# jaxsonpd/air_rs

Hardware: AMD Instinct MI355X
Metric: IQ Msamples/s (decoded Mode-S msgs/s alongside), 2 MSPS i8 stream (higher is better)
Workload: dtype i8; 1 GPU; 2 MSPS i8 IQ, 1 GiB synthetic buffer per GPU, fused magnitude+preamble/DF17 gate+PPM+CRC-24; samples_per_gpu=536870912, bytes_per_gpu=1073741824, channels=1

## Files before the change

### air_rs_amd/csrc/adsb_api.cpp

```cpp
#include <hip/hip_runtime.h>

#include <algorithm>
#include <chrono>
#include <cstdio>
#include <cstdlib>
#include <cmath>
#include <cstring>
#include <new>
#include <vector>

#include "adsb_kernels.h"
#include "adsb_synth.h"

using adsbk::kTile;
using adsbk::kWindow;

namespace {
constexpr int kTimingRing = 512;
}

struct adsb_ctx {
    adsb_cfg cfg{};
    hipStream_t stream = nullptr;
    bool own_stream = false;
// ... 227 lines not shown
        }
        const size_t n_slots = (size_t)c->n_tiles_max * adsbk::kQuota + c->cap_slots;
        bool ok = true;
        for (auto &r : c->rs) {
            ok = ok && hipMalloc((void **)&r.seg, sizeof(adsbk::Seg) * (size_t)c->n_tiles_max) == hipSuccess &&
                 hipMalloc((void **)&r.slots, sizeof(adsb_frame) * n_slots) == hipSuccess &&
                 hipMalloc((void **)&r.out, sizeof(adsb_frame) * (size_t)cfg->max_out) == hipSuccess &&
                 hipMalloc((void **)&r.hdr, sizeof(adsbk::Header)) == hipSuccess &&
                 hipMalloc((void **)&r.chan_prefix, sizeof(uint64_t) * ((size_t)cfg->max_channels + 1)) == hipSuccess &&
                 hipMemsetAsync(r.chan_prefix, 0, sizeof(uint64_t) * ((size_t)cfg->max_channels + 1), c->stream) == hipSuccess &&
                 hipEventCreateWithFlags(&r.k_done, hipEventDisableTiming | hipEventReleaseToDevice) == hipSuccess &&
                 hipEventCreateWithFlags(&r.g_done, hipEventDisableTiming | hipEventReleaseToDevice) == hipSuccess &&
                 hipMemsetAsync(r.hdr, 0, sizeof(adsbk::Header), c->stream) == hipSuccess;
        }
        c->lb_groups_at = (uint32_t)(((size_t)c->n_tiles_max / adsbk::kFinishTilesPerWg + 2 + 63) / 64 * 64);
        const size_t lb_words = (size_t)c->lb_groups_at + c->lb_groups_at / 64 + 64;
        ok = ok && hipMalloc((void **)&c->out_start, sizeof(uint32_t) * ((size_t)c->n_tiles_max + 1)) == hipSuccess &&
             hipMalloc((void **)&c->scratch, 64) == hipSuccess &&
             hipMalloc((void **)&c->lb, sizeof(uint64_t) * lb_words) == hipSuccess &&
             hipMemsetAsync(c->lb, 0, sizeof(uint64_t) * lb_words, c->stream) == hipSuccess &&
             hipMemsetAsync(c->scratch, 0, 64, c->stream) == hipSuccess;
        if (!ok) { fail(ADSB_E_NOMEM); break; }
        if (hipHostMalloc((void **)&c->hdr_host, sizeof(adsbk::Header), hipHostMallocDefault) != hipSuccess) { fail(ADSB_E_NOMEM); break; }
        uint32_t probe[4] = {0, 0, 0, 0};
        e = adsbk::probe_cvt(c->stream, c->scratch, probe);
        if (e != hipSuccess) { fail((int)e); break; }
        const uint32_t want = 0u | (2u << 8) | (180u << 16);
        if (probe[0] == want) c->mag_mode = 0;
        else if (probe[1] == want) c->mag_mode = 1;
        else c->mag_mode = 2;
        if (const char *force = getenv("ADSB_FORCE_MAG_MODE")) c->mag_mode = atoi(force) % 3;
        if (c->scan == adsbk::kScanCode) {
            std::vector<uint16_t> tab(32769);
            const int prc = code_table_check(c, tab.data());
            if (prc != ADSB_OK) { fail(prc); break; }
        }
        c->stamps_bytes = adsbk::tile_stamps_built() ? (size_t)c->n_tiles_max * 64 + 512 : 512;
        if (hipMalloc((void **)&c->stamps, c->stamps_bytes) != hipSuccess || hipMemsetAsync(c->stamps, 0, c->stamps_bytes, c->stream) != hipSuccess) { fail(ADSB_E_NOMEM); break; }
    } while (0);
    if (rc != ADSB_OK) { adsb_destroy(c); return rc; }
    *out_ctx = c;
    return ADSB_OK;
}

extern "C" void *adsb_stream(adsb_ctx *c) { return c ? (void *)c->stream : nullptr; }
extern "C" int adsb_sample_type(const adsb_ctx *c) { return c ? c->cfg.sample_type : ADSB_E_ARG; }
extern "C" int adsb_debug_fused_pass_only(adsb_ctx *c, int on)
{
    if (!c) return ADSB_E_ARG;
    c->fused_pass_only = on != 0;
    return ADSB_OK;
}
extern "C" int adsb_debug_mag_mode(adsb_ctx *c) { return c ? c->mag_mode : ADSB_E_ARG; }
extern "C" int adsb_debug_scan(adsb_ctx *c) { return c ? (c->cfg.sample_type == ADSB_SAMPLE_I8 ? c->scan : adsbk::kScanRoot) : ADSB_E_ARG; }
// ... 1921 lines not shown
```

### air_rs_amd/csrc/adsb_kernels.h

```cpp
#pragma once
#include <hip/hip_runtime.h>
#include <stddef.h>
#include <stdint.h>

#include "../../include/adsb_hip.h"

namespace adsbk {

#ifndef ADSB_KRUN
#define ADSB_KRUN 32
#endif
#ifndef ADSB_THREADS
#define ADSB_THREADS 256
#endif
constexpr int kThreads = ADSB_THREADS;
constexpr int kRun = ADSB_KRUN;
constexpr int kTile = 2 * kThreads * kRun;
constexpr int kHalo = 256;
constexpr int kMag = kTile + kHalo;
#ifndef ADSB_KRUN_I16
#define ADSB_KRUN_I16 16
#endif
constexpr int kRunI16 = ADSB_KRUN_I16;
template <int ST> struct TileCfg {
    static constexpr int kRunT = ST == ADSB_SAMPLE_I8 ? kRun : kRunI16;
    static constexpr int kTileT = 2 * kThreads * kRunT;
    static constexpr int kMagT = kTileT + kHalo;
};
constexpr int tile_offsets(int sample_type)
{
    return sample_type == ADSB_SAMPLE_I8 ? kTile : 2 * kThreads * kRunI16;
}
constexpr int kTileMax = kTile > 2 * kThreads * kRunI16 ? kTile : 2 * kThreads * kRunI16;
constexpr int kScanNsq = 0, kScanRoot = 1, kScanReg = 2, kScanCode = 3, kScanSieve = 4;
constexpr int kRegTile = 4 * 2 * 63 * 32;
#ifndef ADSB_SV_SWEEPS
#define ADSB_SV_SWEEPS 8
#endif
constexpr int kSieveTile = ADSB_SV_SWEEPS * kThreads * 8;
constexpr int tile_offsets_of(int sample_type, int scan)
{
    return (sample_type == ADSB_SAMPLE_I8 && scan == kScanReg) ? kRegTile
           : (sample_type == ADSB_SAMPLE_I8 && scan == kScanSieve) ? kSieveTile : tile_offsets(sample_type);
}
constexpr int kListCap = 128;
constexpr int kSparseCap = 64;
constexpr int kWindow = 240;
constexpr uint32_t kNoBase = 0xFFFFFFFFu;
constexpr uint32_t kQuota = 32;
struct Seg {
    uint32_t base;
    uint32_t cand;
    uint32_t valid;
    uint32_t decoded;
};

struct Header {
    uint64_t n_out;
    uint64_t total_found;
    uint32_t flags;
    uint32_t retry;
    unsigned long long alloc;
};

struct DemodArgs {
    const void *iq;
// ... 19 lines not shown
    Seg *seg;
    adsb_frame *slots;
    adsb_frame *out;
    const uint32_t *out_start;
    uint64_t *lb;
    uint32_t lb_groups_at;
    uint64_t *chan_prefix;
    uint32_t epoch;
    uint32_t tiles_per_channel;
    uint32_t n_channels;
    uint32_t max_out;
    uint32_t tile_first, tile_count;
    Header *hdr;
    uint64_t *hdr_pub;
    uint32_t stall_blk;
};

struct SmallArgs {
    uint32_t *done;
    uint64_t *seq_host;
    uint64_t seq;
};

hipError_t probe_cvt(hipStream_t s, uint32_t *dev_scratch4, uint32_t host_out[4]);
hipError_t launch_code_probe(hipStream_t s, uint16_t *dev_out32769);

hipError_t launch_demod(hipStream_t s, int sample_type, int mag_mode, int scan, const DemodArgs &a,
                        hipEvent_t e0 = nullptr, hipEvent_t e1 = nullptr);
hipError_t launch_finish(hipStream_t s, const FinishArgs &a, hipEvent_t e0 = nullptr, hipEvent_t e1 = nullptr);
hipError_t launch_empty_result(hipStream_t s, Header *hdr, uint64_t *hdr_pub, uint64_t *chan_prefix, uint32_t n_channels,
                               hipEvent_t e0 = nullptr, hipEvent_t e1 = nullptr);
constexpr int kFinishTilesPerWg = 32;
hipError_t launch_small(hipStream_t s, int sample_type, int mag_mode, int scan, const DemodArgs &p, const FinishArgs &f,
                        const SmallArgs &sm);

bool ab_kernels_built();
bool tile_stamps_built();

hipError_t launch_decode_fields(hipStream_t s, const adsb_frame *frames, const Header *hdr, uint32_t cap,
                                adsb_packet_fields *out);

struct TrackRecord {
    adsb_aircraft_record a;
    double t_even, t_odd;
    uint32_t even_lat, even_lon, odd_lat, odd_lon;
    uint32_t have;
    uint32_t pad;
// ... 110 lines not shown
```

### air_rs_amd/csrc/adsb_kernels.hip

```cpp
#include <hip/hip_ext.h>
#include <utility>
#include <cstdlib>

#include "adsb_kernels.h"
#include "adsb_synth.h"

namespace adsbk {

typedef unsigned int u32x4 __attribute__((ext_vector_type(4)));
typedef unsigned short u16x2 __attribute__((ext_vector_type(2)));

__device__ __forceinline__ uint32_t pkmin(uint32_t a, uint32_t b)
{
    u16x2 r = __builtin_elementwise_min(__builtin_bit_cast(u16x2, a), __builtin_bit_cast(u16x2, b));
    return __builtin_bit_cast(uint32_t, r);
}
__device__ __forceinline__ uint32_t pkmax(uint32_t a, uint32_t b)
{
    u16x2 r = __builtin_elementwise_max(__builtin_bit_cast(u16x2, a), __builtin_bit_cast(u16x2, b));
    return __builtin_bit_cast(uint32_t, r);
}
typedef _Float16 f16x2 __attribute__((ext_vector_type(2)));
template <bool F16> __device__ __forceinline__ uint32_t pkmax3(uint32_t a, uint32_t b, uint32_t c)
{
// ... 13 lines not shown
            __builtin_bit_cast(f16x2, c));
        return __builtin_bit_cast(uint32_t, r);
    }
    return pkmin(pkmin(a, b), c);
}

__device__ __forceinline__ void dot4x8_sacc(u32x4 v, int c, int n[8])
{
    const uint32_t a0 = v.x & 0xFFFFu, a1 = v.x & 0xFFFF0000u, a2 = v.y & 0xFFFFu, a3 = v.y & 0xFFFF0000u,
                   a4 = v.z & 0xFFFFu, a5 = v.z & 0xFFFF0000u, a6 = v.w & 0xFFFFu, a7 = v.w & 0xFFFF0000u;
    asm("v_dot4_i32_i8 %0, %8, %12, %20\n\t"
        "v_dot4_i32_i8 %1, %8, %13, %20\n\t"
        "v_dot4_i32_i8 %2, %9, %14, %20\n\t"
        "v_dot4_i32_i8 %3, %9, %15, %20\n\t"
        "v_dot4_i32_i8 %4, %10, %16, %20\n\t"
        "v_dot4_i32_i8 %5, %10, %17, %20\n\t"
        "v_dot4_i32_i8 %6, %11, %18, %20\n\t"
        "v_dot4_i32_i8 %7, %11, %19, %20\n\t"
        "s_nop 2"
        : "=&v"(n[0]), "=&v"(n[1]), "=&v"(n[2]), "=&v"(n[3]), "=&v"(n[4]), "=&v"(n[5]), "=&v"(n[6]), "=&v"(n[7])
        : "v"(v.x), "v"(v.y), "v"(v.z), "v"(v.w), "v"(a0), "v"(a1), "v"(a2), "v"(a3), "v"(a4), "v"(a5),
          "v"(a6), "v"(a7), "s"(c));
}

struct SynTable {
    uint32_t v[112];
};
constexpr SynTable make_syn()
{
    SynTable t{};
    uint32_t r = 1;
    for (int e = 0; e < 112; ++e) {
        t.v[111 - e] = r;
        r <<= 1;
        if (r & 0x1000000u) r ^= 0x1FFF409u;
    }
    return t;
}
__constant__ SynTable kSyn = make_syn();

template <int MAGMODE> __device__ __forceinline__ float mag_root_i8(int n_plus_2p23)
{
    float f = __builtin_bit_cast(float, n_plus_2p23) - 8388607.5f;
    float r = __builtin_amdgcn_sqrtf(f);
    if (MAGMODE == 2) r -= 0.5f;
    return r;
}

typedef float f32x2 __attribute__((ext_vector_type(2)));
template <int MAGMODE>
__device__ __forceinline__ void mags8_i8(u32x4 v, uint32_t &lo, uint32_t &hi)
{
    int n[8];
    dot4x8_sacc(v, 0x4B000000, n);
    float f[8];
#pragma unroll
    for (int k = 0; k < 8; k += 2) {
        f32x2 t = {__builtin_bit_cast(float, n[k]), __builtin_bit_cast(float, n[k + 1])};
        t = t - (f32x2){8388607.5f, 8388607.5f};
        f[k] = t.x;
        f[k + 1] = t.y;
    }
    float r[8];
#pragma unroll
    for (int k = 0; k < 8; ++k) {
        r[k] = __builtin_amdgcn_sqrtf(f[k]);
        if (MAGMODE == 2) r[k] -= 0.5f;
    }
    lo = __builtin_amdgcn_cvt_pk_u8_f32(r[0], 0, 0u);
    lo = __builtin_amdgcn_cvt_pk_u8_f32(r[1], 1, lo);
    lo = __builtin_amdgcn_cvt_pk_u8_f32(r[2], 2, lo);
    lo = __builtin_amdgcn_cvt_pk_u8_f32(r[3], 3, lo);
    hi = __builtin_amdgcn_cvt_pk_u8_f32(r[4], 0, 0u);
    hi = __builtin_amdgcn_cvt_pk_u8_f32(r[5], 1, hi);
    hi = __builtin_amdgcn_cvt_pk_u8_f32(r[6], 2, hi);
    hi = __builtin_amdgcn_cvt_pk_u8_f32(r[7], 3, hi);
}

__device__ __forceinline__ uint32_t mag_i16_fix(uint32_t r, uint32_t n)
{
    return r - ((__umul24(r, r) > n) ? 1u : 0u);
}
__device__ __forceinline__ uint32_t mag_i16(uint32_t iq)
{
    uint32_t n, r;
    asm("v_dot2_i32_i16 %0, %2, %2, 0\n\t"
        "s_nop 2\n\t"
        "v_cvt_f32_u32 %1, %0\n\t"
        "v_sqrt_f32 %1, %1\n\t"
        "s_nop 0\n\t"
        "v_cvt_rpi_i32_f32 %1, %1"
        : "=&v"(n), "=&v"(r)
        : "v"(iq));
    return mag_i16_fix(r, n);
}
__device__ __forceinline__ void mags4_i16(u32x4 v, uint32_t &lo, uint32_t &hi)
{
    uint32_t n0, n1, n2, n3, r0, r1, r2, r3;
    asm("v_dot2_i32_i16 %0, %8, %8, 0\n\t"
// ... 19 lines not shown
        : "v"(v.x), "v"(v.y), "v"(v.z), "v"(v.w));
    lo = __builtin_amdgcn_perm(mag_i16_fix(r1, n1), mag_i16_fix(r0, n0), 0x05040100u);
    hi = __builtin_amdgcn_perm(mag_i16_fix(r3, n3), mag_i16_fix(r2, n2), 0x05040100u);
}

__global__ void probe_cvt_kernel(uint32_t *out)
{
    if (threadIdx.x != 0) return;
    float a = 0.75f, b = 2.5f, c = 180.9986f;
    asm volatile("" : "+v"(a), "+v"(b), "+v"(c));
    uint32_t r0 = __builtin_amdgcn_cvt_pk_u8_f32(a, 0, 0u);
    r0 = __builtin_amdgcn_cvt_pk_u8_f32(b, 1, r0);
    r0 = __builtin_amdgcn_cvt_pk_u8_f32(c, 2, r0);
    out[0] = r0;
    __builtin_amdgcn_s_setreg((1 | (0 << 6) | ((2 - 1) << 11)), 3);
    asm volatile("" : "+v"(a), "+v"(b), "+v"(c));
    uint32_t r1 = __builtin_amdgcn_cvt_pk_u8_f32(a, 0, 0u);
    r1 = __builtin_amdgcn_cvt_pk_u8_f32(b, 1, r1);
    r1 = __builtin_amdgcn_cvt_pk_u8_f32(c, 2, r1);
    out[1] = r1;
    __builtin_amdgcn_s_setreg((1 | (0 << 6) | ((2 - 1) << 11)), 0);
    out[2] = 0xC0DEu;
    out[3] = 0;
}

hipError_t probe_cvt(hipStream_t s, uint32_t *dev_scratch4, uint32_t host_out[4])
{
    hipLaunchKernelGGL(probe_cvt_kernel, dim3(1), dim3(64), 0, s, dev_scratch4);
    hipError_t e = hipGetLastError();
    if (e != hipSuccess) return e;
    e = hipMemcpyAsync(host_out, dev_scratch4, 16, hipMemcpyDeviceToHost, s);
    if (e != hipSuccess) return e;
    return hipStreamSynchronize(s);
}

template <int ST> struct MagT;
template <> struct MagT<ADSB_SAMPLE_I8> { typedef uint8_t type; };
template <> struct MagT<ADSB_SAMPLE_I16> { typedef uint16_t type; };

constexpr int kNsqBias = 72;
constexpr int kNsqHalf = kTile / 2;
constexpr int kNsqLog = kNsqHalf + kHalo;
#ifndef ADSB_NSQ_PAD_SHIFT
#define ADSB_NSQ_PAD_SHIFT 6
#endif
constexpr int kNsqPadShift = ADSB_NSQ_PAD_SHIFT;
__host__ __device__ constexpr uint32_t nsq_phys(uint32_t q) { return q + 4u * (q >> kNsqPadShift); }
constexpr int kNsqPhys = (int)nsq_phys(kNsqLog);
static_assert(kNsqHalf % 64 == 0 && kHalo % 64 == 0 && kRun == 32 && (kNsqPadShift == 5 || kNsqPadShift == 6),
              "nsq image: pads every 32 or 64 dwords, runs of 32");

#ifndef ADSB_MAG_PAD
#define ADSB_MAG_PAD 0
#endif
template <int ST, int SCAN> struct MagPad {
    static constexpr bool on = ADSB_MAG_PAD != 0 && ST == ADSB_SAMPLE_I8 && SCAN == kScanRoot;
};
template <bool PAD> __host__ __device__ constexpr uint32_t mag_phys(uint32_t b) { return PAD ? b + 16u * (b >> 8) : b; }

template <int ST, int SCAN = kScanRoot> struct Lds {
    typedef typename MagT<ST>::type mag_t;
    static constexpr bool kNsq = ST == ADSB_SAMPLE_I8 && SCAN == kScanNsq;
    static constexpr int kMagBytes = kNsq ? kNsqPhys * 4
                                          : (int)((mag_phys<MagPad<ST, SCAN>::on>((uint32_t)TileCfg<ST>::kMagT * (uint32_t)sizeof(mag_t)) + 15u) & ~15u);
    static constexpr int kOffCand = kMagBytes;
    static constexpr int kOffList = kOffCand + 2 * kThreads * 4 * ((TileCfg<ST>::kRunT + 31) / 32);
    static constexpr int kOffMisc = kOffList + kListCap * 2;
    static constexpr int kTotal = kOffMisc + 64;
};

template <int ST>
__device__ __forceinline__ uint32_t pair_at(const uint32_t *ra, const uint32_t *rb, int k)
{
    if (ST == ADSB_SAMPLE_I8) {
        const uint32_t sel = 0x0C000C00u | (uint32_t)(k & 3) | ((uint32_t)(4 + (k & 3)) << 16);
        return __builtin_amdgcn_perm(rb[k >> 2], ra[k >> 2], sel);
    } else {
        const uint32_t sel = (k & 1) ? 0x07060302u : 0x05040100u;
        return __builtin_amdgcn_perm(rb[k >> 1], ra[k >> 1], sel);
    }
}

template <int ST>
__device__ __forceinline__ uint32_t pair_at_cold(const uint32_t *ra, const uint32_t *rb, int k)
{
    if (ST == ADSB_SAMPLE_I8) {
        const uint32_t sel = 0x0C000C00u | (uint32_t)(4 + (k & 3)) | ((uint32_t)(k & 3) << 16);
        return __builtin_amdgcn_perm(ra[k >> 2], rb[k >> 2], sel);
    } else {
// ... 186 lines not shown
#define ADSB_ABL_PHASES 3
#endif
#ifndef ADSB_ABL_NOCMP
#define ADSB_ABL_NOCMP 0
#endif
#ifndef ADSB_AB_KERNELS
#define ADSB_AB_KERNELS 0
#endif
bool ab_kernels_built() { return ADSB_AB_KERNELS != 0; }
#ifndef ADSB_PRIO
#define ADSB_PRIO 0
#endif
#ifndef ADSB_GATE_GROUP
#define ADSB_GATE_GROUP 1
#endif

template <int RUN, int NT>
__device__ __forceinline__ void gate_collect(uint32_t *candA, uint32_t *candB, uint16_t *list, uint32_t *count,
                                             const uint32_t tid, const uint32_t n_valid)
{
    constexpr int WPR = (RUN + 31) / 32;
    const uint32_t sa = tid * RUN, sb = (tid + NT) * RUN;
    const uint32_t va = n_valid > sa ? (n_valid - sa) : 0u, vb = n_valid > sb ? (n_valid - sb) : 0u;
    uint32_t words[2 * WPR];
    uint32_t nz = 0, c = 0;
#pragma unroll
    for (int k = 0; k < WPR; ++k) {
        words[k] = candA[k];
        words[WPR + k] = candB[k];
    }
    if (n_valid < (uint32_t)(2 * NT * RUN)) {
#pragma unroll
        for (int k = 0; k < WPR; ++k) {
            const uint32_t la = va > 32u * k ? va - 32u * k : 0u, lb = vb > 32u * k ? vb - 32u * k : 0u;
            words[k] &= la >= 32u ? 0xFFFFFFFFu : ((1u << la) - 1u);
            words[WPR + k] &= lb >= 32u ? 0xFFFFFFFFu : ((1u << lb) - 1u);
            candA[k] = words[k];
            candB[k] = words[WPR + k];
        }
    }
#pragma unroll
    for (int k = 0; k < 2 * WPR; ++k) {
        nz |= words[k];
        c += __builtin_popcount(words[k]);
    }
    if (nz) {
        uint32_t pos = atomicAdd(count, c);
#pragma unroll
        for (int k = 0; k < 2 * WPR; ++k) {
            uint32_t bits = words[k];
            const uint32_t base = (k < WPR ? sa : sb) + (k % WPR) * 32;
            while (bits) {
                const uint32_t b = __builtin_ctz(bits);
                bits &= bits - 1;
                if (pos < (uint32_t)kSparseCap) list[pos] = (uint16_t)(base + b);
                ++pos;
            }
        }
    }
}

struct NoHook {
    __device__ __forceinline__ void operator()() const {}
};

template <int ST, int GROUP, int RUN, int NT, int HOOK_AT = -1, class HOOK = NoHook, bool F16OK = (ST == ADSB_SAMPLE_I8), bool PAD = false>
__device__ __forceinline__ void gate_phase(const typename MagT<ST>::type *mag, uint32_t *cand, uint16_t *list,
                                           uint32_t *count, const uint32_t tid, const uint32_t n_valid,
                                           HOOK hook = HOOK())
{
    static_assert(RUN % GROUP == 0 && (RUN == 16 || RUN == 32 || RUN == 64), "steps are taken GROUP at a time; 1 or 2 bitmap words per run");
    constexpr int WPR = (RUN + 31) / 32;
    constexpr int SPG = 16 / (int)sizeof(typename MagT<ST>::type);
    uint32_t *candA = cand + WPR * tid, *candB = cand + WPR * (tid + NT);
#pragma unroll
    for (int k = 0; k < WPR; ++k) candA[k] = candB[k] = 0u;
    constexpr int kGran = (RUN + 26 + SPG - 1) / SPG + 1;
    static_assert(!PAD || (ST == ADSB_SAMPLE_I8 && RUN == 32 && (NT * RUN) % 256 == 0), "the padded image: u8 magnitudes, runs of 32 bytes");
    const u32x4 *ga = reinterpret_cast<const u32x4 *>(mag + mag_phys<PAD>(tid * RUN));
    const u32x4 *gb = reinterpret_cast<const u32x4 *>(mag + mag_phys<PAD>((tid + NT) * RUN));
    const uint32_t hop = PAD && (tid & 7u) == 7u ? 1u : 0u;
    const u32x4 *ga2 = ga + hop, *gb2 = gb + hop;
    uint32_t ra[kGran * 4], rb[kGran * 4];
    constexpr int kAhead = 48 / SPG;
#pragma unroll
    for (int g = 0; g < kAhead; ++g) {
        u32x4 a = (PAD && g >= 2) ? ga2[g] : ga[g], b = (PAD && g >= 2) ? gb2[g] : gb[g];
        ra[4 * g] = a.x; ra[4 * g + 1] = a.y; ra[4 * g + 2] = a.z; ra[4 * g + 3] = a.w;
        rb[4 * g] = b.x; rb[4 * g + 1] = b.y; rb[4 * g + 2] = b.z; rb[4 * g + 3] = b.w;
    }

    uint32_t N[RUN + 26], H2[RUN + 8], W3[RUN + 16], F[RUN + 9];
#pragma unroll
    for (int k = 0; k < 25; ++k) N[k] = pair_at<ST>(ra, rb, k);
#pragma unroll
    for (int j = 0; j < 7; ++j) H2[j] = pkmin(N[j], N[j + 2]);
#pragma unroll
    for (int j = 3; j < 13; ++j) W3[j] = pkmax3<F16OK>(N[j], N[j + 1], N[j + 2]);
#pragma unroll
    for (int j = 1; j < 8; ++j) F[j] = pkmax3<F16OK>(N[j], W3[j + 2], N[j + 5]);
// ... 55 lines not shown
    gate_collect<RUN, NT>(candA, candB, list, count, tid, n_valid);
}

template <int BPS, int MAG = kMag>
__device__ __forceinline__ u32x4 tile_rsrc_words(const DemodArgs &p, const TilePos &t, bool live)
{
    const uint64_t base = (uint64_t)(uintptr_t)((const char *)p.iq + ((uint64_t)t.ch * p.channel_stride + t.sample0) * BPS);
    const uint64_t remain = (p.n_samples - t.sample0) * BPS;
    const uint32_t nrec = remain > (uint64_t)(MAG * BPS) ? (uint32_t)(MAG * BPS) : (uint32_t)remain;
    u32x4 w;
    w.x = __builtin_amdgcn_readfirstlane((uint32_t)base);
    w.y = __builtin_amdgcn_readfirstlane((uint32_t)(base >> 32) & 0xFFFFu);
    w.z = __builtin_amdgcn_readfirstlane(live ? nrec : 0u);
    w.w = 0x00020000u;
    return w;
}

#ifndef ADSB_LOAD_AUX
#define ADSB_LOAD_AUX 2
#endif
template <int ST> struct P1 {
    static constexpr int kSPL = ST == ADSB_SAMPLE_I8 ? 8 : 4;
    static constexpr int kIters = (TileCfg<ST>::kMagT + kThreads * kSPL - 1) / (kThreads * kSPL);
};

template <int ST>
__device__ __forceinline__ void issue_tile_loads(const DemodArgs &p, const TilePos &tp, bool live, uint32_t tid,
                                                 u32x4 (&raw)[P1<ST>::kIters])
{
    constexpr int BPS = (ST == ADSB_SAMPLE_I8) ? 2 : 4;
    __amdgpu_buffer_rsrc_t rsrc = tile_rsrc<BPS, TileCfg<ST>::kMagT>(p, tp, live);
    const uint32_t wave_s0 = __builtin_amdgcn_readfirstlane(tid & ~63u) * P1<ST>::kSPL;
#pragma unroll
    for (int it = 0; it < P1<ST>::kIters; ++it)
        if ((uint32_t)it * (kThreads * P1<ST>::kSPL) + wave_s0 < (uint32_t)TileCfg<ST>::kMagT)
            raw[it] = __builtin_amdgcn_raw_buffer_load_b128(rsrc, tid * 16, (uint32_t)it * (kThreads * 16), ADSB_LOAD_AUX);
}

template <int ST, int MAGMODE, bool PAD = false>
__device__ __forceinline__ bool magnitudes_to_lds(const u32x4 (&raw)[P1<ST>::kIters], typename MagT<ST>::type *mag, uint32_t tid)
{
    uint32_t mx = 0;
    const uint32_t wave_s0 = __builtin_amdgcn_readfirstlane(tid & ~63u) * P1<ST>::kSPL;
#pragma unroll
    for (int it = 0; it < P1<ST>::kIters; ++it) {
        if ((uint32_t)it * (kThreads * P1<ST>::kSPL) + wave_s0 < (uint32_t)TileCfg<ST>::kMagT) {
            const uint32_t s = (uint32_t)it * (kThreads * P1<ST>::kSPL) + tid * P1<ST>::kSPL;
            uint32_t lo, hi;
            if (ST == ADSB_SAMPLE_I8) mags8_i8<MAGMODE>(raw[it], lo, hi);
            else {
                mags4_i16(raw[it], lo, hi);
                mx = pkmax(mx, pkmax(lo, hi));
            }
            const uint32_t sp = PAD ? s + 16u * (tid >> 5) + (uint32_t)it * (16u * (kThreads * P1<ST>::kSPL / 256)) : s;
            if (s < (uint32_t)TileCfg<ST>::kMagT) *reinterpret_cast<uint2 *>(mag + sp) = make_uint2(lo, hi);
        }
    }
    return ST == ADSB_SAMPLE_I16 && __builtin_amdgcn_ballot_w64(((mx & 0xFFFFu) >= 0x7C00u) || ((mx >> 16) >= 0x7C00u)) != 0;
}

constexpr int kNsqIters = (kNsqLog + kThreads * 8 - 1) / (kThreads * 8);
constexpr int kNsqFull = kNsqLog / (kThreads * 8);
constexpr int kNsqTail = kNsqLog % (kThreads * 8);
static_assert(kNsqIters - kNsqFull <= 1 && kNsqTail % 8 == 0, "at most one partial sweep of whole lanes");

__device__ __forceinline__ void nsq_issue_loads(const DemodArgs &p, const TilePos &tp, uint32_t tid,
                                                u32x4 (&ra)[kNsqIters], u32x4 (&rb)[kNsqIters])
{
    __amdgpu_buffer_rsrc_t rsrc = tile_rsrc<2, kMag>(p, tp, true);
#pragma unroll
    for (int it = 0; it < kNsqFull; ++it) {
        ra[it] = __builtin_amdgcn_raw_buffer_load_b128(rsrc, tid * 16, (uint32_t)it * (kThreads * 16), ADSB_LOAD_AUX);
        rb[it] = __builtin_amdgcn_raw_buffer_load_b128(rsrc, tid * 16, (uint32_t)it * (kThreads * 16) + 2 * kNsqHalf, ADSB_LOAD_AUX);
    }
    if (kNsqTail && __builtin_amdgcn_readfirstlane(tid & ~63u) * 8 < (uint32_t)kNsqTail) {
        ra[kNsqFull] = __builtin_amdgcn_raw_buffer_load_b128(rsrc, tid * 16, (uint32_t)kNsqFull * (kThreads * 16), ADSB_LOAD_AUX);
        rb[kNsqFull] = __builtin_amdgcn_raw_buffer_load_b128(rsrc, tid * 16, (uint32_t)kNsqFull * (kThreads * 16) + 2 * kNsqHalf, ADSB_LOAD_AUX);
    }
// ... 124 lines not shown
                uint32_t bit = 1u << o;
                asm("" : "+v"(bit));
                if (sa) atomicOr(candA, bit);
                if (sb) atomicOr(candB, bit);
            }
        }
    }
    gate_collect<RUN, NT>(candA, candB, list, count, tid, n_valid);
}

#ifndef ADSB_SCAN_WAVES
#define ADSB_SCAN_WAVES 4
#endif
#ifndef ADSB_REG_ABL
#define ADSB_REG_ABL 0
#endif
#ifndef ADSB_REG_WAVES
#define ADSB_REG_WAVES 5
#endif
template <int ST, int MAGMODE, int SCAN>
__device__ __forceinline__ void scan_tile(const DemodArgs &p, const uint32_t tile, const bool first, unsigned char *smem)
{
    typedef Lds<ST, SCAN> L;
    typedef TileCfg<ST> TC;
    typedef typename L::mag_t mag_t;
    constexpr bool NSQ = L::kNsq;
    static_assert(kThreads / 64 <= 4, "misc[4 + wave] must stay below misc[8]");

    mag_t *mag = reinterpret_cast<mag_t *>(smem);
    uint32_t *img = reinterpret_cast<uint32_t *>(smem);
    uint32_t *cand = reinterpret_cast<uint32_t *>(smem + L::kOffCand);
    uint16_t *list = reinterpret_cast<uint16_t *>(smem + L::kOffList);
    uint32_t *misc = reinterpret_cast<uint32_t *>(smem + L::kOffMisc);

    const uint32_t tid = threadIdx.x;
    const uint32_t lane = tid & 63, wave = tid >> 6;

#if ADSB_PRIO & 1
    __builtin_amdgcn_s_setprio(3);
#endif
    if (!NSQ && MAGMODE == 1) __builtin_amdgcn_s_setreg((1 | (0 << 6) | ((2 - 1) << 11)), 3);
#if ADSB_TILE_STAMPS
    unsigned long long ts_prev = 0;
    uint32_t ts_seg[9] = {0, 0, 0, 0, 0, 0, 0, 0, 0};
    ts_seg[7] = (uint32_t)__builtin_amdgcn_s_memrealtime();
    TSTAMP(-1);
    ts_seg[8] = (uint32_t)ts_prev;
// ... 29 lines not shown
        if constexpr (NSQ) wave_big = nsq_image_to_lds(raw_a, raw_b, img, tid);
        else wave_big = magnitudes_to_lds<ST, MAGMODE, MagPad<ST, SCAN>::on>(raw, mag, tid);
        if ((NSQ || ST == ADSB_SAMPLE_I16) && lane == 0) misc[4 + wave] = wave_big ? 1u : 0u;
        TSTAMP(1);
        __syncthreads();
        TSTAMP(2);
#if ADSB_ABL_PHASES < 2
        if (smem[tid * 64] == 0xFD && smem[tid * 64 + 1] == 0xFE && n_valid == 7) misc[12] = 1;
#else

        if constexpr (NSQ || ST == ADSB_SAMPLE_I16) {
            uint32_t any_big = 0;
#pragma unroll
            for (int w = 0; w < kThreads / 64; ++w) any_big |= misc[4 + w];
            const bool big = any_big != 0;
            if constexpr (NSQ) {
                if (!big) gate_phase_nsq<true>(img, cand, list, &misc[12], tid, n_valid);
                else gate_phase_nsq<false>(img, cand, list, &misc[12], tid, n_valid);
            } else {
                if (!big) gate_phase<ST, ADSB_GATE_GROUP, TC::kRunT, kThreads, -1, NoHook, true>(mag, cand, list, &misc[12], tid, n_valid);
                else gate_phase<ST, ADSB_GATE_GROUP, TC::kRunT, kThreads, -1, NoHook, false>(mag, cand, list, &misc[12], tid, n_valid);
            }
        } else {
            gate_phase<ST, ADSB_GATE_GROUP, TC::kRunT, kThreads, -1, NoHook, (ST == ADSB_SAMPLE_I8), MagPad<ST, SCAN>::on>(mag, cand, list, &misc[12], tid, n_valid);
        }
#endif
        TSTAMP(3);
        __syncthreads();
        TSTAMP(4);

#if ADSB_PRIO & 2
        __builtin_amdgcn_s_setprio(2);
#endif
        uint32_t total = misc[12];
#if ADSB_ABL_PHASES < 3
        if (total != 0x7FFFFFFFu) total = 0;
#endif
        const bool dense = total > (uint32_t)kSparseCap;
        constexpr int kBitsPerWord = TC::kRunT < 32 ? TC::kRunT : 32;
        u32x4 cw = {0, 0, 0, 0};
        uint32_t cnt = 0, my_first = 0;
        if (dense) {
            if (4 * tid < (uint32_t)(TC::kTileT / kBitsPerWord)) cw = reinterpret_cast<const u32x4 *>(cand)[tid];
            cnt = __builtin_popcount(cw.x) + __builtin_popcount(cw.y) + __builtin_popcount(cw.z) +
                  __builtin_popcount(cw.w);
            uint32_t incl = cnt;
#pragma unroll
// ... 1236 lines not shown
        *sm.done = 0;
        __builtin_amdgcn_fence(__ATOMIC_RELEASE, "");
        asm volatile("s_waitcnt vmcnt(0)" ::: "memory");
        __hip_atomic_store(sm.seq_host, sm.seq, __ATOMIC_RELAXED, __HIP_MEMORY_SCOPE_SYSTEM);
    }
}

hipError_t launch_small(hipStream_t s, int sample_type, int mag_mode, int scan, const DemodArgs &p, const FinishArgs &f,
                        const SmallArgs &sm)
{
    if (p.tile_count == 0 || p.tile_count > (uint32_t)kFinTiles) return hipErrorInvalidValue;
    dim3 grid(p.tile_count), block(kThreads);
    if (sample_type == ADSB_SAMPLE_I16) hipLaunchKernelGGL((demod_small<ADSB_SAMPLE_I16, 0, kScanRoot>), grid, block, 0, s, p, f, sm);
#if ADSB_AB_KERNELS
    else if (scan == kScanSieve) hipLaunchKernelGGL((demod_small<ADSB_SAMPLE_I8, 0, kScanSieve>), grid, block, 0, s, p, f, sm);
    else if (scan == kScanNsq) hipLaunchKernelGGL((demod_small<ADSB_SAMPLE_I8, 0, kScanNsq>), grid, block, 0, s, p, f, sm);
    else if (scan == kScanReg) hipLaunchKernelGGL((demod_small<ADSB_SAMPLE_I8, 0, kScanReg>), grid, block, 0, s, p, f, sm);
    else if (scan == kScanCode) hipLaunchKernelGGL((demod_small<ADSB_SAMPLE_I8, 0, kScanCode>), grid, block, 0, s, p, f, sm);
#else
    else if (scan != kScanRoot) return hipErrorInvalidValue;
#endif
    else if (mag_mode == 0) hipLaunchKernelGGL((demod_small<ADSB_SAMPLE_I8, 0, kScanRoot>), grid, block, 0, s, p, f, sm);
    else if (mag_mode == 1) hipLaunchKernelGGL((demod_small<ADSB_SAMPLE_I8, 1, kScanRoot>), grid, block, 0, s, p, f, sm);
    else hipLaunchKernelGGL((demod_small<ADSB_SAMPLE_I8, 2, kScanRoot>), grid, block, 0, s, p, f, sm);
    return hipGetLastError();
}

__global__ void empty_result_kernel(Header *hdr, uint64_t *hdr_pub, uint64_t *chan_prefix, uint32_t n_channels)
{
    if (threadIdx.x == 0) {
        hdr->n_out = 0;
        hdr->total_found = 0;
        hdr->flags = 0;
        hdr->retry = 0;
        hdr->alloc = 0;
        if (hdr_pub) { hdr_pub[0] = 0; hdr_pub[1] = 0; hdr_pub[2] = 0; hdr_pub[3] = 0; }
    }
    if (chan_prefix)
        for (uint32_t k = threadIdx.x; k <= n_channels; k += blockDim.x) chan_prefix[k] = 0;
}
hipError_t launch_empty_result(hipStream_t s, Header *hdr, uint64_t *hdr_pub, uint64_t *chan_prefix, uint32_t n_channels,
                               hipEvent_t e0, hipEvent_t e1)
{
    hipExtLaunchKernelGGL(empty_result_kernel, dim3(1), dim3(64), 0, s, e0, e1, 0, hdr, hdr_pub, chan_prefix, n_channels);
    return hipGetLastError();
}

template <int ST>
static hipError_t launch_demod_st(hipStream_t s, int mag_mode, const DemodArgs &a, uint32_t grid_x,
                                  hipEvent_t e0, hipEvent_t e1)
{
    dim3 grid(grid_x), block(kThreads);
    if (ST == ADSB_SAMPLE_I16) mag_mode = 0;
    switch (mag_mode) {
    case 0: hipExtLaunchKernelGGL((demod_tiles<ST, 0, kScanRoot>), grid, block, 0, s, e0, e1, 0, a); break;
    case 1: hipExtLaunchKernelGGL((demod_tiles<ST, ST == ADSB_SAMPLE_I8 ? 1 : 0, kScanRoot>), grid, block, 0, s, e0, e1, 0, a); break;
    default: hipExtLaunchKernelGGL((demod_tiles<ST, ST == ADSB_SAMPLE_I8 ? 2 : 0, kScanRoot>), grid, block, 0, s, e0, e1, 0, a); break;
    }
    return hipGetLastError();
}

bool tile_stamps_built() { return ADSB_TILE_STAMPS != 0; }

hipError_t launch_demod(hipStream_t s, int sample_type, int mag_mode, int scan, const DemodArgs &a,
                        hipEvent_t e0, hipEvent_t e1)
{
    if (a.tile_count == 0) return hipSuccess;
#if ADSB_AB_KERNELS
    if (sample_type == ADSB_SAMPLE_I8 && scan == kScanSieve) {
        uint32_t grid = a.tile_count;
        if (kSievePersistent) {
            static int sieve_slots = 0;
            if (sieve_slots == 0) {
                int dev = 0, cus = 0;
                if (hipGetDevice(&dev) != hipSuccess || hipDeviceGetAttribute(&cus, hipDeviceAttributeMultiprocessorCount, dev) != hipSuccess || cus <= 0) cus = 256;
                sieve_slots = cus * 4;
            }
            if (grid > (uint32_t)sieve_slots) grid = (uint32_t)sieve_slots;
        }
// ... 96 lines not shown
            mags8_i8<MAGMODE>(v, lo, hi);
            for (int k = 0; k < 8; ++k)
                if (g * 8 + k < n) out[g * 8 + k] = (uint16_t)(((k < 4 ? lo : hi) >> (8 * (k & 3))) & 0xFFu);
        }
    } else {
        const uint32_t *src = reinterpret_cast<const uint32_t *>(iq);
        for (size_t k = (size_t)blockIdx.x * blockDim.x + threadIdx.x; k < n; k += stride)
            out[k] = (uint16_t)mag_i16(src[k]);
    }
    if (MAGMODE == 1) __builtin_amdgcn_s_setreg((1 | (0 << 6) | ((2 - 1) << 11)), 0);
}

hipError_t launch_magnitudes(hipStream_t s, int sample_type, int mag_mode, const void *iq, size_t n,
                             uint16_t *out)
{
    if (n == 0) return hipSuccess;
    dim3 grid(1024), block(256);
    if (sample_type == ADSB_SAMPLE_I16) {
        hipLaunchKernelGGL((magnitudes_kernel<ADSB_SAMPLE_I16, 0>), grid, block, 0, s, iq, n, out);
    } else if (mag_mode == 0) {
        hipLaunchKernelGGL((magnitudes_kernel<ADSB_SAMPLE_I8, 0>), grid, block, 0, s, iq, n, out);
    } else if (mag_mode == 1) {
        hipLaunchKernelGGL((magnitudes_kernel<ADSB_SAMPLE_I8, 1>), grid, block, 0, s, iq, n, out);
    } else {
        hipLaunchKernelGGL((magnitudes_kernel<ADSB_SAMPLE_I8, 2>), grid, block, 0, s, iq, n, out);
    }
    return hipGetLastError();
}

__global__ void nsq_values_kernel(const void *iq, size_t n, uint16_t *out)
{
    const size_t stride = (size_t)gridDim.x * blockDim.x;
    const size_t groups = (n + 7) / 8;
    for (size_t g = (size_t)blockIdx.x * blockDim.x + threadIdx.x; g < groups; g += stride) {
        const uint16_t *src = reinterpret_cast<const uint16_t *>(iq) + g * 8;
        uint16_t tmp[8];
        for (int k = 0; k < 8; ++k) tmp[k] = (g * 8 + k < n) ? src[k] : (uint16_t)0;
        u32x4 v;
        v.x = tmp[0] | ((uint32_t)tmp[1] << 16);
        v.y = tmp[2] | ((uint32_t)tmp[3] << 16);
        v.z = tmp[4] | ((uint32_t)tmp[5] << 16);
        v.w = tmp[6] | ((uint32_t)tmp[7] << 16);
        uint32_t d[8];
        nsq_pack16(v, v, d);
        for (int k = 0; k < 8; ++k)
            if (g * 8 + k < n) out[g * 8 + k] = (d[k] & 0xFFFFu) == (d[k] >> 16) ? (uint16_t)(d[k] & 0xFFFFu) : (uint16_t)0xFFFFu;
// ... 87 lines not shown
```

Baseline: 2.670 million Msamples/s.

## Add packed f16 magnitude mode and shrink root-scan tile to 252 gate lanes

Result: slower. 2.612 million Msamples/s (-2.2%).

```diff
diff --git a/air_rs_amd/csrc/adsb_api.cpp b/air_rs_amd/csrc/adsb_api.cpp
--- a/air_rs_amd/csrc/adsb_api.cpp
+++ b/air_rs_amd/csrc/adsb_api.cpp
@@ -273,14 +273,15 @@
              hipMemsetAsync(c->scratch, 0, 64, c->stream) == hipSuccess;
         if (!ok) { fail(ADSB_E_NOMEM); break; }
         if (hipHostMalloc((void **)&c->hdr_host, sizeof(adsbk::Header), hipHostMallocDefault) != hipSuccess) { fail(ADSB_E_NOMEM); break; }
-        uint32_t probe[4] = {0, 0, 0, 0};
+        uint32_t probe[8] = {0, 0, 0, 0, 0, 0, 0, 0};
         e = adsbk::probe_cvt(c->stream, c->scratch, probe);
         if (e != hipSuccess) { fail((int)e); break; }
-        const uint32_t want = 0u | (2u << 8) | (180u << 16);
-        if (probe[0] == want) c->mag_mode = 0;
-        else if (probe[1] == want) c->mag_mode = 1;
+        const char *pair = getenv("ADSB_MAG_PAIR");
+        if (probe[4] == adsbk::kProbePairLo && probe[5] == adsbk::kProbePairHi && !(pair && atoi(pair) == 0)) c->mag_mode = 3;
+        else if (probe[0] == adsbk::kProbeU8Want) c->mag_mode = 0;
+        else if (probe[1] == adsbk::kProbeU8Want) c->mag_mode = 1;
         else c->mag_mode = 2;
-        if (const char *force = getenv("ADSB_FORCE_MAG_MODE")) c->mag_mode = atoi(force) % 3;
+        if (const char *force = getenv("ADSB_FORCE_MAG_MODE")) c->mag_mode = atoi(force) & 3;
         if (c->scan == adsbk::kScanCode) {
             std::vector<uint16_t> tab(32769);
             const int prc = code_table_check(c, tab.data());
diff --git a/air_rs_amd/csrc/adsb_kernels.h b/air_rs_amd/csrc/adsb_kernels.h
--- a/air_rs_amd/csrc/adsb_kernels.h
+++ b/air_rs_amd/csrc/adsb_kernels.h
@@ -22,9 +22,18 @@
 #define ADSB_KRUN_I16 16
 #endif
 constexpr int kRunI16 = ADSB_KRUN_I16;
-template <int ST> struct TileCfg {
+#ifndef ADSB_ROOT_LANES
+#define ADSB_ROOT_LANES 252
+#endif
+constexpr int kRootLanes = ADSB_ROOT_LANES;
+constexpr int kRootTile = 2 * kRootLanes * kRun;
+static_assert(kRootLanes <= kThreads && kRootLanes >= kThreads - 4 && kRootLanes % 4 == 0,
+              "idle gate lanes park their bitmap words in the spare words behind the tile's; the dense path reads four words per lane");
+constexpr int kScanNsq = 0, kScanRoot = 1, kScanReg = 2, kScanCode = 3, kScanSieve = 4;
+template <int ST, int SCAN = kScanRoot> struct TileCfg {
     static constexpr int kRunT = ST == ADSB_SAMPLE_I8 ? kRun : kRunI16;
-    static constexpr int kTileT = 2 * kThreads * kRunT;
+    static constexpr int kLanesT = (ST == ADSB_SAMPLE_I8 && SCAN == kScanRoot) ? kRootLanes : kThreads;
+    static constexpr int kTileT = 2 * kLanesT * kRunT;
     static constexpr int kMagT = kTileT + kHalo;
 };
 constexpr int tile_offsets(int sample_type)
@@ -32,7 +41,6 @@
     return sample_type == ADSB_SAMPLE_I8 ? kTile : 2 * kThreads * kRunI16;
 }
 constexpr int kTileMax = kTile > 2 * kThreads * kRunI16 ? kTile : 2 * kThreads * kRunI16;
-constexpr int kScanNsq = 0, kScanRoot = 1, kScanReg = 2, kScanCode = 3, kScanSieve = 4;
 constexpr int kRegTile = 4 * 2 * 63 * 32;
 #ifndef ADSB_SV_SWEEPS
 #define ADSB_SV_SWEEPS 8
@@ -41,7 +49,8 @@
 constexpr int tile_offsets_of(int sample_type, int scan)
 {
     return (sample_type == ADSB_SAMPLE_I8 && scan == kScanReg) ? kRegTile
-           : (sample_type == ADSB_SAMPLE_I8 && scan == kScanSieve) ? kSieveTile : tile_offsets(sample_type);
+           : (sample_type == ADSB_SAMPLE_I8 && scan == kScanSieve) ? kSieveTile
+           : (sample_type == ADSB_SAMPLE_I8 && scan == kScanRoot) ? kRootTile : tile_offsets(sample_type);
 }
 constexpr int kListCap = 128;
 constexpr int kSparseCap = 64;
@@ -107,7 +116,10 @@
     uint64_t seq;
 };
 
-hipError_t probe_cvt(hipStream_t s, uint32_t *dev_scratch4, uint32_t host_out[4]);
+constexpr uint32_t kProbeU8Want = 0u | (2u << 8) | (180u << 16);
+constexpr uint32_t kProbePairLo = 0u | (1u << 8) | (1u << 16) | (2u << 24);
+constexpr uint32_t kProbePairHi = 180u | (181u << 8) | (181u << 16) | (181u << 24);
+hipError_t probe_cvt(hipStream_t s, uint32_t *dev_scratch8, uint32_t host_out[8]);
 hipError_t launch_code_probe(hipStream_t s, uint16_t *dev_out32769);
 
 hipError_t launch_demod(hipStream_t s, int sample_type, int mag_mode, int scan, const DemodArgs &a,
diff --git a/air_rs_amd/csrc/adsb_kernels.hip b/air_rs_amd/csrc/adsb_kernels.hip
--- a/air_rs_amd/csrc/adsb_kernels.hip
+++ b/air_rs_amd/csrc/adsb_kernels.hip
@@ -59,6 +59,47 @@
         : "v"(v.x), "v"(v.y), "v"(v.z), "v"(v.w), "v"(a0), "v"(a1), "v"(a2), "v"(a3), "v"(a4), "v"(a5),
           "v"(a6), "v"(a7), "s"(c));
 }
+#ifndef ADSB_P1_COVER
+#define ADSB_P1_COVER 1
+#endif
+__device__ __forceinline__ void masks8(u32x4 v, uint32_t (&a)[8])
+{
+    a[0] = v.x & 0xFFFFu, a[1] = v.x & 0xFFFF0000u, a[2] = v.y & 0xFFFFu, a[3] = v.y & 0xFFFF0000u;
+    a[4] = v.z & 0xFFFFu, a[5] = v.z & 0xFFFF0000u, a[6] = v.w & 0xFFFFu, a[7] = v.w & 0xFFFF0000u;
+}
+__device__ __forceinline__ void dot4x4_then_masks(uint32_t v0, uint32_t v1, uint32_t nv0, uint32_t nv1, int c, int *n, uint32_t *a)
+{
+    asm("v_dot4_i32_i8 %0, %8, %4, %12\n\t"
+        "v_dot4_i32_i8 %1, %8, %5, %12\n\t"
+        "v_dot4_i32_i8 %2, %9, %6, %12\n\t"
+        "v_dot4_i32_i8 %3, %9, %7, %12\n\t"
+        "v_and_b32 %4, %13, %10\n\t"
+        "v_and_b32 %5, %14, %10\n\t"
+        "v_and_b32 %6, %13, %11\n\t"
+        "v_and_b32 %7, %14, %11"
+        : "=&v"(n[0]), "=&v"(n[1]), "=&v"(n[2]), "=&v"(n[3]), "+v"(a[0]), "+v"(a[1]), "+v"(a[2]), "+v"(a[3])
+        : "v"(v0), "v"(v1), "v"(nv0), "v"(nv1), "s"(c), "s"(0xFFFFu), "s"(0xFFFF0000u));
+}
+__device__ __forceinline__ void dot4x8_then_masks(u32x4 v, u32x4 next, int c, int n[8], uint32_t (&a)[8])
+{
+    dot4x4_then_masks(v.x, v.y, next.x, next.y, c, n, a);
+    dot4x4_then_masks(v.z, v.w, next.z, next.w, c, n + 4, a + 4);
+}
+__device__ __forceinline__ void dot4x8_masked(u32x4 v, const uint32_t (&a)[8], int c, int n[8])
+{
+    asm("v_dot4_i32_i8 %0, %8, %12, %20\n\t"
+        "v_dot4_i32_i8 %1, %8, %13, %20\n\t"
+        "v_dot4_i32_i8 %2, %9, %14, %20\n\t"
+        "v_dot4_i32_i8 %3, %9, %15, %20\n\t"
+        "v_dot4_i32_i8 %4, %10, %16, %20\n\t"
+        "v_dot4_i32_i8 %5, %10, %17, %20\n\t"
+        "v_dot4_i32_i8 %6, %11, %18, %20\n\t"
+        "v_dot4_i32_i8 %7, %11, %19, %20\n\t"
+        "s_nop 2"
+        : "=&v"(n[0]), "=&v"(n[1]), "=&v"(n[2]), "=&v"(n[3]), "=&v"(n[4]), "=&v"(n[5]), "=&v"(n[6]), "=&v"(n[7])
+        : "v"(v.x), "v"(v.y), "v"(v.z), "v"(v.w), "v"(a[0]), "v"(a[1]), "v"(a[2]), "v"(a[3]), "v"(a[4]), "v"(a[5]),
+          "v"(a[6]), "v"(a[7]), "s"(c));
+}
 
 struct SynTable {
     uint32_t v[112];
@@ -85,11 +126,22 @@
 }
 
 typedef float f32x2 __attribute__((ext_vector_type(2)));
+constexpr float kTwoM48 = 0x1p-48f;
+__device__ __forceinline__ uint32_t mag_pair_f16(int n0_plus_2p23, int n1_plus_2p23)
+{
+    f32x2 t = {__builtin_bit_cast(float, n0_plus_2p23), __builtin_bit_cast(float, n1_plus_2p23)};
+    t = __builtin_elementwise_fma(t, (f32x2){kTwoM48, kTwoM48}, (f32x2){-8388607.5f * kTwoM48, -8388607.5f * kTwoM48});
+    return __builtin_bit_cast(uint32_t, __builtin_amdgcn_cvt_pkrtz(__builtin_amdgcn_sqrtf(t.x), __builtin_amdgcn_sqrtf(t.y)));
+}
+
 template <int MAGMODE>
-__device__ __forceinline__ void mags8_i8(u32x4 v, uint32_t &lo, uint32_t &hi)
-{
-    int n[8];
-    dot4x8_sacc(v, 0x4B000000, n);
+__device__ __forceinline__ void roots8_i8(const int (&n)[8], uint32_t &lo, uint32_t &hi)
+{
+    if (MAGMODE == 3) {
+        lo = __builtin_amdgcn_perm(mag_pair_f16(n[2], n[3]), mag_pair_f16(n[0], n[1]), 0x06040200u);
+        hi = __builtin_amdgcn_perm(mag_pair_f16(n[6], n[7]), mag_pair_f16(n[4], n[5]), 0x06040200u);
+        return;
+    }
     float f[8];
 #pragma unroll
     for (int k = 0; k < 8; k += 2) {
@@ -112,6 +164,14 @@
     hi = __builtin_amdgcn_cvt_pk_u8_f32(r[5], 1, hi);
     hi = __builtin_amdgcn_cvt_pk_u8_f32(r[6], 2, hi);
     hi = __builtin_amdgcn_cvt_pk_u8_f32(r[7], 3, hi);
+}
+
+template <int MAGMODE>
+__device__ __forceinline__ void mags8_i8(u32x4 v, uint32_t &lo, uint32_t &hi)
+{
+    int n[8];
+    dot4x8_sacc(v, 0x4B000000, n);
+    roots8_i8<MAGMODE>(n, lo, hi);
 }
 
 __device__ __forceinline__ uint32_t mag_i16_fix(uint32_t r, uint32_t n)
@@ -177,14 +237,21 @@
     __builtin_amdgcn_s_setreg((1 | (0 << 6) | ((2 - 1) << 11)), 0);
     out[2] = 0xC0DEu;
     out[3] = 0;
-}
-
-hipError_t probe_cvt(hipStream_t s, uint32_t *dev_scratch4, uint32_t host_out[4])
-{
-    hipLaunchKernelGGL(probe_cvt_kernel, dim3(1), dim3(64), 0, s, dev_scratch4);
+    int n[8] = {0, 1, 3, 4, 32760, 32761, 32768, 32768};
+#pragma unroll
+    for (int k = 0; k < 8; ++k) {
+        n[k] += 0x4B000000;
+        asm volatile("" : "+v"(n[k]));
+    }
+    roots8_i8<3>(n, out[4], out[5]);
+}
+
+hipError_t probe_cvt(hipStream_t s, uint32_t *dev_scratch8, uint32_t host_out[8])
+{
+    hipLaunchKernelGGL(probe_cvt_kernel, dim3(1), dim3(64), 0, s, dev_scratch8);
     hipError_t e = hipGetLastError();
     if (e != hipSuccess) return e;
-    e = hipMemcpyAsync(host_out, dev_scratch4, 16, hipMemcpyDeviceToHost, s);
+    e = hipMemcpyAsync(host_out, dev_scratch8, 32, hipMemcpyDeviceToHost, s);
     if (e != hipSuccess) return e;
     return hipStreamSynchronize(s);
 }
@@ -217,9 +284,11 @@
     typedef typename MagT<ST>::type mag_t;
     static constexpr bool kNsq = ST == ADSB_SAMPLE_I8 && SCAN == kScanNsq;
     static constexpr int kMagBytes = kNsq ? kNsqPhys * 4
-                                          : (int)((mag_phys<MagPad<ST, SCAN>::on>((uint32_t)TileCfg<ST>::kMagT * (uint32_t)sizeof(mag_t)) + 15u) & ~15u);
+                                          : (int)((mag_phys<MagPad<ST, SCAN>::on>((uint32_t)TileCfg<ST, SCAN>::kMagT * (uint32_t)sizeof(mag_t)) + 15u) & ~15u);
     static constexpr int kOffCand = kMagBytes;
-    static constexpr int kOffList = kOffCand + 2 * kThreads * 4 * ((TileCfg<ST>::kRunT + 31) / 32);
+    static constexpr int kCandWords = (TileCfg<ST, SCAN>::kLanesT < kThreads ? kThreads + 2 * TileCfg<ST, SCAN>::kLanesT : 2 * kThreads) *
+                                      ((TileCfg<ST, SCAN>::kRunT + 31) / 32);
+    static constexpr int kOffList = kOffCand + 4 * kCandWords;
     static constexpr int kOffMisc = kOffList + kListCap * 2;
     static constexpr int kTotal = kOffMisc + 64;
 };
@@ -452,12 +521,13 @@
     constexpr int WPR = (RUN + 31) / 32;
     const uint32_t sa = tid * RUN, sb = (tid + NT) * RUN;
     const uint32_t va = n_valid > sa ? (n_valid - sa) : 0u, vb = n_valid > sb ? (n_valid - sb) : 0u;
+    const bool idle = NT < kThreads && tid >= (uint32_t)NT;
     uint32_t words[2 * WPR];
     uint32_t nz = 0, c = 0;
 #pragma unroll
     for (int k = 0; k < WPR; ++k) {
-        words[k] = candA[k];
-        words[WPR + k] = candB[k];
+        words[k] = idle ? 0u : candA[k];
+        words[WPR + k] = idle ? 0u : candB[k];
     }
     if (n_valid < (uint32_t)(2 * NT * RUN)) {
 #pragma unroll
@@ -502,10 +572,14 @@
     static_assert(RUN % GROUP == 0 && (RUN == 16 || RUN == 32 || RUN == 64), "steps are taken GROUP at a time; 1 or 2 bitmap words per run");
     constexpr int WPR = (RUN + 31) / 32;
     constexpr int SPG = 16 / (int)sizeof(typename MagT<ST>::type);
-    uint32_t *candA = cand + WPR * tid, *candB = cand + WPR * (tid + NT);
+    const uint32_t ctid = (NT < kThreads && tid >= (uint32_t)NT) ? tid + NT : tid;
+    uint32_t *candA = cand + WPR * ctid, *candB = candA + WPR * NT;
+    
 #pragma unroll
     for (int k = 0; k < WPR; ++k) candA[k] = candB[k] = 0u;
     constexpr int kGran = (RUN + 26 + SPG - 1) / SPG + 1;
+    static_assert(NT >= kThreads || (!PAD && (kThreads - 1 + NT) * RUN + kGran * SPG <= 2 * NT * RUN + kHalo),
+                  "idle lanes read inside the image");
     static_assert(!PAD || (ST == ADSB_SAMPLE_I8 && RUN == 32 && (NT * RUN) % 256 == 0), "the padded image: u8 magnitudes, runs of 32 bytes");
     const u32x4 *ga = reinterpret_cast<const u32x4 *>(mag + mag_phys<PAD>(tid * RUN));
     const u32x4 *gb = reinterpret_cast<const u32x4 *>(mag + mag_phys<PAD>((tid + NT) * RUN));
@@ -607,6 +681,7 @@
 template <int ST> struct P1 {
     static constexpr int kSPL = ST == ADSB_SAMPLE_I8 ? 8 : 4;
     static constexpr int kIters = (TileCfg<ST>::kMagT + kThreads * kSPL - 1) / (kThreads * kSPL);
+    static constexpr int kWhole = ST == ADSB_SAMPLE_I8 ? TileCfg<ST>::kMagT / (kThreads * kSPL) : 0;
 };
 
 template <int ST>
@@ -618,7 +693,7 @@
     const uint32_t wave_s0 = __builtin_amdgcn_readfirstlane(tid & ~63u) * P1<ST>::kSPL;
 #pragma unroll
     for (int it = 0; it < P1<ST>::kIters; ++it)
-        if ((uint32_t)it * (kThreads * P1<ST>::kSPL) + wave_s0 < (uint32_t)TileCfg<ST>::kMagT)
+        if (it < P1<ST>::kWhole || (uint32_t)it * (kThreads * P1<ST>::kSPL) + wave_s0 < (uint32_t)TileCfg<ST>::kMagT)
             raw[it] = __builtin_amdgcn_raw_buffer_load_b128(rsrc, tid * 16, (uint32_t)it * (kThreads * 16), ADSB_LOAD_AUX);
 }
 
@@ -627,9 +702,25 @@
 {
     uint32_t mx = 0;
     const uint32_t wave_s0 = __builtin_amdgcn_readfirstlane(tid & ~63u) * P1<ST>::kSPL;
-#pragma unroll
-    for (int it = 0; it < P1<ST>::kIters; ++it) {
-        if ((uint32_t)it * (kThreads * P1<ST>::kSPL) + wave_s0 < (uint32_t)TileCfg<ST>::kMagT) {
+    constexpr int kChain = (ST == ADSB_SAMPLE_I8 && MAGMODE == 3 && ADSB_P1_COVER) ? P1<ST>::kWhole : 0;
+    if constexpr (kChain > 0) {
+        uint32_t a[8];
+        masks8(raw[0], a);
+#pragma unroll
+        for (int it = 0; it < kChain; ++it) {
+            int n[8];
+            if (it + 1 < kChain) dot4x8_then_masks(raw[it], raw[it + 1], 0x4B000000, n, a);
+            else dot4x8_masked(raw[it], a, 0x4B000000, n);
+            uint32_t lo, hi;
+            roots8_i8<MAGMODE>(n, lo, hi);
+            const uint32_t s = (uint32_t)it * (kThreads * P1<ST>::kSPL) + tid * P1<ST>::kSPL;
+            const uint32_t sp = PAD ? s + 16u * (tid >> 5) + (uint32_t)it * (16u * (kThreads * P1<ST>::kSPL / 256)) : s;
+            *reinterpret_cast<uint2 *>(mag + sp) = make_uint2(lo, hi);
+        }
+    }
+#pragma unroll
+    for (int it = kChain; it < P1<ST>::kIters; ++it) {
+        if (it < P1<ST>::kWhole || (uint32_t)it * (kThreads * P1<ST>::kSPL) + wave_s0 < (uint32_t)TileCfg<ST>::kMagT) {
             const uint32_t s = (uint32_t)it * (kThreads * P1<ST>::kSPL) + tid * P1<ST>::kSPL;
             uint32_t lo, hi;
             if (ST == ADSB_SAMPLE_I8) mags8_i8<MAGMODE>(raw[it], lo, hi);
@@ -638,7 +729,7 @@
                 mx = pkmax(mx, pkmax(lo, hi));
             }
             const uint32_t sp = PAD ? s + 16u * (tid >> 5) + (uint32_t)it * (16u * (kThreads * P1<ST>::kSPL / 256)) : s;
-            if (s < (uint32_t)TileCfg<ST>::kMagT) *reinterpret_cast<uint2 *>(mag + sp) = make_uint2(lo, hi);
+            if (it < P1<ST>::kWhole || s < (uint32_t)TileCfg<ST>::kMagT) *reinterpret_cast<uint2 *>(mag + sp) = make_uint2(lo, hi);
         }
     }
     return ST == ADSB_SAMPLE_I16 && __builtin_amdgcn_ballot_w64(((mx & 0xFFFFu) >= 0x7C00u) || ((mx >> 16) >= 0x7C00u)) != 0;
@@ -809,7 +900,7 @@
 __device__ __forceinline__ void scan_tile(const DemodArgs &p, const uint32_t tile, const bool first, unsigned char *smem)
 {
     typedef Lds<ST, SCAN> L;
-    typedef TileCfg<ST> TC;
+    typedef TileCfg<ST, SCAN> TC;
     typedef typename L::mag_t mag_t;
     constexpr bool NSQ = L::kNsq;
     static_assert(kThreads / 64 <= 4, "misc[4 + wave] must stay below misc[8]");
@@ -885,7 +976,7 @@
                 else gate_phase<ST, ADSB_GATE_GROUP, TC::kRunT, kThreads, -1, NoHook, false>(mag, cand, list, &misc[12], tid, n_valid);
             }
         } else {
-            gate_phase<ST, ADSB_GATE_GROUP, TC::kRunT, kThreads, -1, NoHook, (ST == ADSB_SAMPLE_I8), MagPad<ST, SCAN>::on>(mag, cand, list, &misc[12], tid, n_valid);
+            gate_phase<ST, ADSB_GATE_GROUP, TC::kRunT, TC::kLanesT, -1, NoHook, (ST == ADSB_SAMPLE_I8), MagPad<ST, SCAN>::on>(mag, cand, list, &misc[12], tid, n_valid);
         }
 #endif
         TSTAMP(3);
@@ -2168,6 +2259,7 @@
 #endif
     else if (mag_mode == 0) hipLaunchKernelGGL((demod_small<ADSB_SAMPLE_I8, 0, kScanRoot>), grid, block, 0, s, p, f, sm);
     else if (mag_mode == 1) hipLaunchKernelGGL((demod_small<ADSB_SAMPLE_I8, 1, kScanRoot>), grid, block, 0, s, p, f, sm);
+    else if (mag_mode == 3) hipLaunchKernelGGL((demod_small<ADSB_SAMPLE_I8, 3, kScanRoot>), grid, block, 0, s, p, f, sm);
     else hipLaunchKernelGGL((demod_small<ADSB_SAMPLE_I8, 2, kScanRoot>), grid, block, 0, s, p, f, sm);
     return hipGetLastError();
 }
@@ -2201,6 +2293,7 @@
     switch (mag_mode) {
     case 0: hipExtLaunchKernelGGL((demod_tiles<ST, 0, kScanRoot>), grid, block, 0, s, e0, e1, 0, a); break;
     case 1: hipExtLaunchKernelGGL((demod_tiles<ST, ST == ADSB_SAMPLE_I8 ? 1 : 0, kScanRoot>), grid, block, 0, s, e0, e1, 0, a); break;
+    case 3: hipExtLaunchKernelGGL((demod_tiles<ST, ST == ADSB_SAMPLE_I8 ? 3 : 0, kScanRoot>), grid, block, 0, s, e0, e1, 0, a); break;
     default: hipExtLaunchKernelGGL((demod_tiles<ST, ST == ADSB_SAMPLE_I8 ? 2 : 0, kScanRoot>), grid, block, 0, s, e0, e1, 0, a); break;
     }
     return hipGetLastError();
@@ -2343,6 +2436,8 @@
         hipLaunchKernelGGL((magnitudes_kernel<ADSB_SAMPLE_I8, 0>), grid, block, 0, s, iq, n, out);
     } else if (mag_mode == 1) {
         hipLaunchKernelGGL((magnitudes_kernel<ADSB_SAMPLE_I8, 1>), grid, block, 0, s, iq, n, out);
+    } else if (mag_mode == 3) {
+        hipLaunchKernelGGL((magnitudes_kernel<ADSB_SAMPLE_I8, 3>), grid, block, 0, s, iq, n, out);
     } else {
         hipLaunchKernelGGL((magnitudes_kernel<ADSB_SAMPLE_I8, 2>), grid, block, 0, s, iq, n, out);
     }
```
